# rubengooj/stvo-pl

Hardware: AMD Instinct MI355X
Metric: stereo frames/s (match+optimizePose) (higher is better)
Workload: dtype u8/fp4+f64; 1 GPU; BASELINE configs[2]: KITTI-00-shaped stereo with points + lines (ORB + LBD rows), grid-windowed stereo match (points and lines) + f2f brute-force mutual-NNR match (points and lines) + full GN optimizePose (config_kitti.yaml), device-resident per-frame pipeline; the streams cycle through the 8 sequence ids / 3 KITTI calibrations of configs[4] (sequence s on rank s mod G); streams_per_gpu=3072, parallelism=seq-shard x1

## Files before the change

stvo-pl_amd/csrc/debug_switches.h:

```cpp
#pragma once

#include <climits>

namespace stvo {

constexpr int DBG_UNSET = INT_MIN;

struct DebugSwitches {
    int pose_kernel;
    int pose2p_nw;
    int pose_prof;
    int pose_los;
    int knn_mfma;
    int knn_nseg;
    int seq_inline;
    int line_fused;
    int match_small;
    int match_lazy;
    int grid_tail;
    int grid_fused;
    int grid_fused_cap;
    int lsd_grow;
    int lsd_waves;
    int lsd_xcd_blocks;
    int lsd_feed_ahead;
    int lsd_sep;
    int lsd_multi;
    int lsd_ahead;
    int cells_ahead;
    int lines_ahead;
    int grid_cells;
};

const DebugSwitches& dbg();
void dbg_reparse();

}
```

stvo-pl_amd/csrc/kernels.h:

```cpp
#pragma once

#include <hip/hip_runtime.h>
#include <stdint.h>

#include <cstdlib>
#include <map>
#include <mutex>
#include <utility>

#include "../../include/stvo_hip.h"
#include "debug_switches.h"
#include "point_tail.h"

namespace stvo {

inline bool lds_opt_in(const void* kernel, int bytes) {
    static std::mutex mu;
    static std::map<std::pair<const void*, int>, int> granted;
    int dev = 0;
    if (hipGetDevice(&dev) != hipSuccess) return false;
    std::lock_guard<std::mutex> lk(mu);
    const auto key = std::make_pair(kernel, dev);
    const auto it = granted.find(key);
    if (it != granted.end() && (it->second >= bytes || it->second < 0)) return it->second >= bytes;
// ... 103 lines not shown
    double level_scale;
    const unsigned* wait_flag;
    unsigned wait_value;
    int lazy_eig;
    int lines_on_solver;
    const uint4* fetch_src;
    uint4* fetch_dst;
    unsigned fetch_n16;
    unsigned* fetch_flag;
    unsigned fetch_value;
    unsigned* start_flag;
    unsigned start_value;
};
bool pose_start_flag_ok(const PoseArgs& a);
void launch_stream_gate(hipStream_t s, const unsigned* flag, unsigned value);
constexpr int STVO_POSE_QTAB = 16;
constexpr int PATH_EIG_PENDING = 1 << 30;
bool pose_inline_sync_ok(int B);
void launch_stream_signal(hipStream_t s, unsigned* flag, unsigned value);
int launch_pose(hipStream_t s, const PoseArgs& a);
int launch_pose2p(hipStream_t s, const PoseArgs& a);
bool pose_batch_kernel_selected(const PoseArgs& a);
int pose2p_waves_per_pair(int B);
void pose2p_retain_stream(hipStream_t s);
void pose2p_release_stream(hipStream_t s);

void launch_blur7_u8(hipStream_t s, int B, int cols, int rows, const uint8_t* src, uint8_t* dst, const int* k7);
void launch_resize_linear_u8(hipStream_t s, int B, int scols, int srows, int dcols, int drows, const uint8_t* src, uint8_t* dst, double fx = 0.0,
                             double fy = 0.0);

constexpr int GRID_LW = STVO_GRID_COLS + 16, GRID_LCELLS = STVO_GRID_ROWS * GRID_LW, GRID_LSTART_STRIDE = GRID_LCELLS + 4;
struct PointCells {
    int K, ws;
    const float* kp_l;
    const float* kp_r;
    const int32_t* n_kp_l;
    const int32_t* n_kp_r;
    const double* inv_wh;
    int32_t* pstart;
    uint32_t* plstart;
    int32_t* plperm;
    int32_t* pperm;
    int32_t* pcell;
    int32_t* pxy_l;
    unsigned long long* top2_p;
    int32_t* govf_p;
// ... 60 lines not shown
```

stvo-pl_amd/csrc/pose_block.h:

```cpp
#pragma once
#include <type_traits>

#include "kernels.h"
#include "pose_math.h"

namespace stvo {

namespace {

constexpr int ACT_CONTINUE = 0, ACT_BREAK = 1, ACT_FAIL = 2;

struct PoseSh {
    double DT[16];
    double DT0[16];
    double DT1[16];
    double DTr[16];
    double cov[36];
    double eig[6];
    double H[36];
    double g[6];
    double err, err_prev, err_out, lambda;
    double s_p, s_l;
    unsigned long long xchg[2];
    int action, good, n_inl_p, n_inl_l, n_m_p, n_m_l, evals, itmp;
// ... 195 lines not shown
            const unsigned olo = (unsigned)k_or, ohi = (unsigned)((unsigned long long)k_or >> 32);
            const unsigned a0 = (unsigned)__builtin_amdgcn_update_dpp((int)alo, (int)alo, CTRL, RM, 0xf, false);
            const unsigned a1 = (unsigned)__builtin_amdgcn_update_dpp((int)ahi, (int)ahi, CTRL, RM, 0xf, false);
            const unsigned o0 = (unsigned)__builtin_amdgcn_update_dpp((int)olo, (int)olo, CTRL, RM, 0xf, false);
            const unsigned o1 = (unsigned)__builtin_amdgcn_update_dpp((int)ohi, (int)ohi, CTRL, RM, 0xf, false);
            k_and &= (K)(((unsigned long long)a1 << 32) | a0);
            k_or |= (K)(((unsigned long long)o1 << 32) | o0);
        };
        using std::integral_constant;
        dpp_step(integral_constant<int, 0x111>{}, integral_constant<int, 0xf>{});
        dpp_step(integral_constant<int, 0x112>{}, integral_constant<int, 0xf>{});
        dpp_step(integral_constant<int, 0x114>{}, integral_constant<int, 0xf>{});
        dpp_step(integral_constant<int, 0x118>{}, integral_constant<int, 0xf>{});
        dpp_step(integral_constant<int, 0x142>{}, integral_constant<int, 0xa>{});
        dpp_step(integral_constant<int, 0x143>{}, integral_constant<int, 0xc>{});
        if ((threadIdx.x & 63) == 63) {
            part[0] = (unsigned long long)k_and;
            part[1] = (unsigned long long)k_or;
        }
    }

    template <int NA, int NB, bool W, typename K, int BITS, typename KeyA, typename KeyB>
    static __device__ __forceinline__ void select2(KeyA&& ka, unsigned ma, int ktha, bool acta, KeyB&& kb, unsigned mb, int kthb, bool actb,
                                                   unsigned* S, unsigned long long* xchg, int& rot, K& outa, K& outb, bool sc = false) {
        static_assert(BITS == 32 || BITS == 64, "32- or 64-bit keys");
        const int tid = threadIdx.x, wv = tid >> 6;
        const bool own_b = W ? !sc : sc;
        constexpr bool PFA = BITS == 64 && NA >= 8, PFB = BITS == 64 && NB >= 8;
        K anda = 0, ora = ~(K)0, andb = 0, orb = ~(K)0;
        if (PFA || PFB) {
            unsigned long long* part = reinterpret_cast<unsigned long long*>(S + SEL_PART);
            if (W) {
                if (PFA) sel_and_or<NA, K>(ka, ma, part + 4 * wv);
                if (PFB && !sc) sel_and_or<NB, K>(kb, mb, part + 4 * wv + 2);
            }
            __syncthreads();
            unsigned long long a0 = ~0ull, o0 = 0ull, a1 = ~0ull, o1 = 0ull;
#pragma unroll
            for (int w = 0; w < NWORK; ++w) {
                if (PFA) { a0 &= part[4 * w]; o0 |= part[4 * w + 1]; }
                if (PFB) { a1 &= part[4 * w + 2]; o1 |= part[4 * w + 3]; }
            }
            if (PFA) { anda = (K)a0; ora = (K)o0; }
            if (PFB && !sc) { andb = (K)a1; orb = (K)o1; }
        }
        auto top_bit = [](K differ) -> int {
            return differ == 0 ? -1 : (BITS - 1) - (BITS == 64 ? __clzll((unsigned long long)differ) : __clz((unsigned)differ));
        };
        K pa = anda, pb = andb;
        int kka = ktha, kkb = kthb;
        int hia = acta ? top_bit(anda ^ ora) : -1, hib = actb ? top_bit(andb ^ orb) : -1;
        bool penda = false, pendb = false;
        auto count = [&](auto n_c, auto&& key, unsigned mask, K prefix, int hi, int lo, unsigned* h) {
            constexpr int N = decltype(n_c)::value;
#pragma unroll
            for (int k = 0; k < N; ++k) {
                const K kv = key(k);
                const K diff = kv ^ prefix;
                const bool same = hi + 1 >= BITS ? true : (diff >> (hi + 1 >= BITS ? 0 : hi + 1)) == 0;
// ... 9 lines not shown
            prefix = (prefix & ~((K)127 << lo)) | ((K)bin << lo);
            kk -= below;
            hi = lo - 1;
            if (cnt == 1 && lo > 0) {
                if (own) {
#pragma unroll
                    for (int k = 0; k < N; ++k) {
                        const K kv = key(k);
                        if (((mask >> k) & 1u) && ((kv ^ prefix) >> lo) == 0) *mail = (unsigned long long)kv;
                    }
                }
                pend = true;
                hi = -1;
            }
        };
        using std::integral_constant;
        while (hia >= 0 || hib >= 0) {
            const int loa = hia >= 6 ? hia - 6 : 0, lob = hib >= 6 ? hib - 6 : 0;
            unsigned* const ha = S + rot * SEL_HW;
            unsigned* const hb = S + (3 + rot) * SEL_HW;
            if (W && hia >= 0) count(integral_constant<int, NA>{}, ka, ma, pa, hia, loa, ha);
            if (own_b && hib >= 0) count(integral_constant<int, NB>{}, kb, mb, pb, hib, lob, hb);
            __syncthreads();
            if (W && tid < 2 * SEL_HW) {
                const int rc = rot == 0 ? 2 : rot - 1;
                S[((tid >> 6) * 3 + rc) * SEL_HW + (tid & 63)] = 0u;
            }
            if (hia >= 0) decide(integral_constant<int, NA>{}, W, ka, ma, ha, pa, kka, hia, loa, penda, xchg);
            if (hib >= 0) decide(integral_constant<int, NB>{}, own_b, kb, mb, hb, pb, kkb, hib, lob, pendb, xchg + 1);
            rot = rot == 2 ? 0 : rot + 1;
        }
        __syncthreads();
        if (penda) pa = (K)xchg[0];
        if (pendb) pb = (K)xchg[1];
        if (acta) outa = pa;
        if (actb) outb = pb;
    }

    template <int NA, int NB, bool W>
    static __device__ __forceinline__ void mad_sigma2(const double* va, unsigned ma, int na, const double* vb, unsigned mb, int nb, unsigned* S,
                                                      unsigned long long* xchg, int& rot, double& sa, double& sb, bool sc = false) {
        sa = 0.0;
        sb = 0.0;
        const bool acta = na != 0, actb = nb != 0;
        if (!acta && !actb) return;
        auto image = [](double v) -> unsigned long long {
            const unsigned long long b = (unsigned long long)__double_as_longlong(v);
            return (b >> 63) ? ~b : (b | 0x8000000000000000ull);
        };
        auto value = [](unsigned long long k) -> double {
            return __longlong_as_double((long long)((k >> 63) ? (k & 0x7FFFFFFFFFFFFFFFull) : ~k));
        };
        unsigned long long ra = 0ull, rb = 0ull;
        select2<NA, NB, W, unsigned long long, 64>([&](int k) { return image(va[k]); }, ma, na / 2, acta, [&](int k) { return image(vb[k]); }, mb,
                                                   nb / 2, actb, S, xchg, rot, ra, rb, sc);
        const double meda = value(ra), medb = value(rb);
        unsigned qa = 0u, qb = 0u;
        select2<NA, NB, W, unsigned, 32>([&](int k) { return __float_as_uint(fabsf((float)(va[k] - meda))); }, ma, na / 2, acta,
                                         [&](int k) { return __float_as_uint(fabsf((float)(vb[k] - medb))); }, mb, nb / 2, actb, S, xchg, rot, qa, qb, sc);
        if (acta) sa = 1.4826 * (double)__uint_as_float(qa);
        if (actb) sb = 1.4826 * (double)__uint_as_float(qb);
    }

    template <int N, bool W>
    static __device__ __forceinline__ void sum_at(const double* v, double (*red)[28], int slot0, double* out, bool sc = false) {
        const int lane = threadIdx.x & 63, wv = W ? (int)(threadIdx.x >> 6) : NW;
        if (W || sc) {
#pragma unroll
            for (int k = 0; k < N; ++k) {
                const double s = wave_sum_lane63(v[k]);
                if (lane == 63) red[wv][slot0 + k] = s;
            }
        }
        __syncthreads();
#pragma unroll
        for (int k = 0; k < N; ++k) {
            double s = red[0][slot0 + k];
#pragma unroll
            for (int w = 1; w < NW; ++w) s += red[w][slot0 + k];
            if (sc) s += red[NW][slot0 + k];
            out[k] = s;
        }
    }

    template <int NA, int NB, bool W>
    static __device__ __forceinline__ void outlier_cut(const double* ra, unsigned ma, int na, bool do_a, const double* rb, unsigned mb, int nb,
                                                       bool do_b, double inlier_k, unsigned& inla, unsigned& inlb, unsigned* S,
                                                       unsigned long long* xchg, int& rot, double (*red)[28], int* cnt, bool sc = false) {
        const bool own_b = W ? !sc : sc;
        double sa, sb;
        mad_sigma2<NA, NB, W>(ra, do_a ? ma : 0u, do_a ? na : 0, rb, do_b ? mb : 0u, do_b ? nb : 0, S, xchg, rot, sa, sb, sc);
        double v[6] = {0.0, 0.0, 0.0, 0.0, 0.0, 0.0};
        if (W) {
#pragma unroll
            for (int k = 0; k < NA; ++k)
                if (do_a && ((ma >> k) & 1u)) {
                    if (ra[k] < 2.0 * sa) {
                        v[0] += ra[k];
                        v[1] += 1.0;
                    }
                    v[2] += ra[k];
                }
        }
        if (own_b) {
#pragma unroll
            for (int k = 0; k < NB; ++k)
                if (do_b && ((mb >> k) & 1u)) {
                    if (rb[k] < 2.0 * sb) {
                        v[3] += rb[k];
                        v[4] += 1.0;
                    }
                    v[5] += rb[k];
                }
        }
// ... 176 lines not shown
    for (int i = 0; i < 36; ++i) C[i] = sh->cov[i];
    pm::eig6_ql(C, w);
#pragma unroll
    for (int i = 0; i < 6; ++i) sh->eig[i] = w[i];
    sh->good = pm::is_good_solution(DT, w, err) ? 1 : 0;
}

__device__ __forceinline__ void t0_is_good_fast(PoseSh* sh, const double* DT, double err) {
    if (err < 0.0 || err > 1.0 || !pm::all_finite16(DT)) {
        sh->good = 0;
        return;
    }
    double C[36];
#pragma unroll
    for (int i = 0; i < 36; ++i) C[i] = sh->cov[i];
    if (pm::spd_unit_certificate(C) == 1) {
        sh->good = 1;
        return;
    }
    t0_is_good(sh, DT, err);
}

__device__ __forceinline__ void t0_commit(PoseSh* sh, stvo_pose_result* out, int status, int path, int it0, int it1, bool lazy_eig = false,
                                          double* next_T = nullptr) {
    bool eig_pending = false;
    if (lazy_eig) {
        double C[36];
#pragma unroll
        for (int i = 0; i < 36; ++i) C[i] = sh->cov[i];
        if (sh->err_out < 0.0 || sh->err_out > 1.0 || !pm::all_finite16(sh->DT)) {
            sh->good = 0;
        } else if (pm::spd_unit_certificate(C) == 1) {
            sh->good = 1;
            eig_pending = true;
        } else {
            t0_is_good(sh, sh->DT, sh->err_out);
        }
    } else {
        t0_is_good(sh, sh->DT, sh->err_out);
    }
    double DT[16];
#pragma unroll
    for (int i = 0; i < 16; ++i) {
        DT[i] = sh->DT[i];
        out->T_opt[i] = DT[i];
    }
    out->err_opt = sh->err_out;
    if (sh->good && !pm::is_identity16(DT)) {
        double Ti[16], x[6], T[16];
        pm::inverse_se3(DT, Ti);
        pm::logmap_se3(Ti, x);
        pm::expmap_se3(x, T);
#pragma unroll
        for (int i = 0; i < 16; ++i) out->T[i] = T[i];
        if (next_T) {
            const bool fin = pm::all_finite16(T);
#pragma unroll
            for (int i = 0; i < 16; ++i) next_T[i] = fin ? T[i] : ((i % 5 == 0) ? 1.0 : 0.0);
        }
#pragma unroll
        for (int i = 0; i < 36; ++i) out->cov[i] = sh->cov[i];
#pragma unroll
        for (int i = 0; i < 6; ++i) out->cov_eig[i] = eig_pending ? 0.0 : sh->eig[i];
// ... 132 lines not shown
```

stvo-pl_amd/csrc/pose_kernel2p.hip:

```cpp
#include <cstdlib>

#include <map>
#include <mutex>
#include <utility>
#include <vector>

#include "pose_block.h"

namespace stvo {
namespace {

__device__ __forceinline__ double uni(double v) {
    const long long b = __double_as_longlong(v);
    const int lo = __builtin_amdgcn_readfirstlane((int)(b & 0xFFFFFFFFll)), hi = __builtin_amdgcn_readfirstlane((int)(b >> 32));
    return __longlong_as_double(((long long)hi << 32) | (unsigned long long)(unsigned)lo);
}

struct PointRec2 {
    double X, Y, Z, ox, oy, q;
};

constexpr bool POSE2P_PRIO = true;

template <int NW, bool PROF>
// ... 415 lines not shown
    KArgs* const kargs = (KArgs*)__builtin_amdgcn_kernarg_segment_ptr();
    auto ka = [&]() -> KArgs& {
        KArgs* p = kargs;
        asm volatile("" : "+s"(p));
        return *p;
    };

    constexpr int BLOCK = NW * 64;
    constexpr int PPT = (STVO_POSE_MAX_POINTS + BLOCK - 1) / BLOCK;
    constexpr int LPT = (STVO_POSE_MAX_LINES + BLOCK - 1) / BLOCK;
    constexpr int KL = pose2c_planes<NW>();
    constexpr bool HAS_REG = KL < PPT;
    static_assert(KL <= PPT && PPT <= 16, "4-bit levels of 16 ordinals in one 64-bit word");
    using Ops = BlockOps<NW>;
    extern __shared__ float4 s_ra[];
    double* const s_rb = reinterpret_cast<double*>(s_ra + KL * BLOCK);
    __shared__ __align__(16) int s_hist[2][Ops::HIST_W];
    __shared__ double s_red[NW][28];
    __shared__ int s_ired[NW];
    __shared__ PoseSh s_sh;
    PoseSh* sh = &s_sh;
    const int f = blockIdx.x, tid = threadIdx.x, lane = tid & 63, wv = tid >> 6;
    const bool w0 = wv == 0, t0 = tid == 0;
    long long rprof[3] = {0, 0, 0};
    long long tprof[5] = {0, 0, 0, 0, 0};
    long long wprof[3] = {0, 0, 0}, wave_busy = 0;
    auto tick = [&]() -> long long {
        if constexpr (PROF) return (long long)__builtin_readcyclecounter();
        else return 0ll;
    };
    const long long t_begin = tick();
    if (blockIdx.x == 0 && threadIdx.x == 0 && ka().start_flag)
        __hip_atomic_store(ka().start_flag, ka().start_value, __ATOMIC_RELEASE, __HIP_MEMORY_SCOPE_AGENT);
    stvo_cam cam_f;
    if (ka().cams) {
        cam_f = ka().cams[f];
    } else {
        cam_f.fx = ka().cam.fx; cam_f.fy = ka().cam.fy; cam_f.cx = ka().cam.cx; cam_f.cy = ka().cam.cy; cam_f.b = ka().cam.b;
    }
    const pm::Cam5 cam{cam_f.fx, cam_f.fy, cam_f.cx, cam_f.cy};
    const double cam_b = cam_f.b;
    const double homog_th = ka().prm.homog_th, inv_homog = 1.0 / homog_th;

    unsigned pmatched = 0u, pinl = 0u;
    const int n_prev_p = ka().n_prev_pts != nullptr ? min(ka().n_prev_pts[f], ka().max_pts) : 0;
    const size_t pbase = (size_t)f * ka().max_pts;
    int jj[PPT];
// ... 27 lines not shown
        int initl[LPT];
#pragma unroll
        for (int k = 0; k < LPT; ++k) {
            const int li = li0 + k * BLOCK;
            const int lc = (li < n_prev_l && li < ka().max_lines) ? li : 0;
            jl[k] = (ka().m12l && ka().max_lines > 0) ? ka().m12l[lbase + lc] : lc;
            initl[k] = (ka().init_inl_l && ka().max_lines > 0) ? ka().init_inl_l[lbase + lc] : 1;
        }
#pragma unroll
        for (int k = 0; k < LPT; ++k) {
            const int li = li0 + k * BLOCK;
            if (li < n_prev_l && li < ka().max_lines && jl[k] >= 0) {
                lmatched |= 1u << k;
                if (initl[k] != 0) linl |= 1u << k;
            } else {
                jl[k] = 0;
            }
        }
    }
    const int n_mine = __popc(pmatched);
    unsigned* const sel = reinterpret_cast<unsigned*>(&s_hist[0][0]);
    int sel_rot = 0;
    for (int i = tid; i < 2 * Ops::HIST_W; i += BLOCK) sel[i] = 0u;
    const int n_m_p = Ops::template sum_int<true>(n_mine, s_ired);
    const int n_m_l = Ops::template sum_int<true>(__popc(lmatched), s_ired);

    const unsigned m_o = n_mine >= 32 ? 0xFFFFFFFFu : ((1u << n_mine) - 1u);
    unsigned inl_o = 0u, slow_o = 0u;
    unsigned long long lv = 0ull;
    float4 xa = make_float4(0.f, 0.f, 0.f, 0.f);
    double xb = 1.0;
    {
        int r = 0;
        constexpr int STAGE_CH = PPT;
#pragma unroll
        for (int k0 = 0; k0 < PPT; k0 += STAGE_CH) {
            float4 pv[STAGE_CH], cv[STAGE_CH];
#pragma unroll
            for (int c = 0; c < STAGE_CH; ++c) {
                const int k = k0 + c;
                if (k >= PPT) continue;
                const int ik = tid + k * BLOCK;
                pv[c] = ka().prev_rc[pbase + (size_t)(ik < n_prev_p ? ik : 0)];
                cv[c] = ka().curr_rc[pbase + (size_t)jj[k]];
            }
#pragma unroll
            for (int c = 0; c < STAGE_CH; ++c) {
                const int k = k0 + c;
// ... 35 lines not shown
        const double2 v0 = q[0], v1 = q[BLOCK], v2 = q[2 * BLOCK], v3 = q[3 * BLOCK], v4 = q[4 * BLOCK], v5 = q[5 * BLOCK], v6 = q[6 * BLOCK];
        L.sP[0] = v0.x; L.sP[1] = v0.y; L.sP[2] = v1.x; L.eP[0] = v1.y; L.eP[1] = v2.x; L.eP[2] = v2.y;
        L.le[0] = v3.x; L.le[1] = v3.y; L.le[2] = v4.x; L.spl[0] = v4.y; L.spl[1] = v5.x; L.epl[0] = v5.y; L.epl[1] = v6.x;
        L.sigma2 = v6.y;
        return L;
    };
#pragma unroll
    for (int k = 0; k < LPT; ++k)
        if ((lmatched >> k) & 1u) {
            const size_t i = lbase + (size_t)(li0 + k * BLOCK);
            const size_t j = lbase + (size_t)jl[k];
            const int r = __popc(lmatched & ((1u << k) - 1u));
            double2* q = ar_l + (size_t)(r * 7) * BLOCK + tid;
            q[0] = make_double2(ka().prev_sP[i * 3 + 0], ka().prev_sP[i * 3 + 1]);
            q[BLOCK] = make_double2(ka().prev_sP[i * 3 + 2], ka().prev_eP[i * 3 + 0]);
            q[2 * BLOCK] = make_double2(ka().prev_eP[i * 3 + 1], ka().prev_eP[i * 3 + 2]);
            q[3 * BLOCK] = make_double2(ka().curr_le[j * 3 + 0], ka().curr_le[j * 3 + 1]);
            q[4 * BLOCK] = make_double2(ka().curr_le[j * 3 + 2], ka().prev_spl[i * 2 + 0]);
            q[5 * BLOCK] = make_double2(ka().prev_spl[i * 2 + 1], ka().prev_epl[i * 2 + 0]);
            q[6 * BLOCK] = make_double2(ka().prev_epl[i * 2 + 1], sqrt(ka().prev_s2l[i]));
        }

    {
        const int nip = Ops::template sum_int<true>(__popc(inl_o), s_ired);
        const int nil = Ops::template sum_int<true>(__popc(linl), s_ired);
        if (w0) {
            sh->n_m_p = n_m_p;
            sh->n_m_l = n_m_l;
            sh->n_inl_p = nip;
            sh->n_inl_l = nil;
            sh->good = 1;
            sh->err_out = -1.0;
#pragma unroll
            for (int i = 0; i < 16; ++i) {
                const double v = ka().init_T ? ka().init_T[(size_t)f * 16 + i] : ((i % 5 == 0) ? 1.0 : 0.0);
                sh->DT[i] = v;
                sh->DT0[i] = v;
            }
#pragma unroll
            for (int i = 0; i < 36; ++i) {
                sh->cov[i] = 0.0;
                sh->H[i] = 0.0;
            }
        }
        __syncthreads();
    }
    const long long t_prologue = tick() - t_begin;

    auto rebuild = [&](const float4& av, double bd, double* X, double* Y, double* Z, double* ox, double* oy) {
#pragma clang fp contract(off)
        *X = bd * ((double)av.x - cam_f.cx);
        *Y = bd * ((double)av.y - cam_f.cy);
        *Z = bd * cam_f.fx;
        *ox = (double)av.z;
        *oy = (double)av.w;
    };
    const double* const qtab = ka().q_tab;
    auto q_of = [&](unsigned nib) -> double { return qtab[nib]; };
    auto fetch_slow = [&](int r) -> CompactRec {
        return pose2c_fetch_slow(ka().prev_rc, ka().curr_rc, ka().m12p, pbase, tid, BLOCK, pmatched, r, cam_b, ka().level_scale);
// ... 109 lines not shown
        wave_busy += tw2 - tw0;
        __syncthreads();
        if (w0) {
            if (lane < 28) {
                double sum = s_red[0][lane];
#pragma unroll
                for (int w = 1; w < NW; ++w) sum += s_red[w][lane];
                store_total(sh, lane, sum);
            }
            __builtin_amdgcn_fence(__ATOMIC_RELEASE, "wavefront");
            __builtin_amdgcn_wave_barrier();
            __builtin_amdgcn_fence(__ATOMIC_ACQUIRE, "wavefront");
        }
        wprof[0] += tw1 - tw0;
        wprof[1] += tw2 - tw1;
        wprof[2] += tick() - tw2;
    };

    auto compact_inliers = [&]() {
        unsigned char* const s_lvb = reinterpret_cast<unsigned char*>(&s_hist[0][0]);
        static_assert(sizeof(s_hist) >= (size_t)KL * BLOCK, "the level bytes of a full set of planes fit the histogram scratch");
        const unsigned mov = inl_o & ~slow_o;
        const int c = __popc(mov);
        int incl = c;
#pragma unroll
        for (int off = 1; off < 64; off <<= 1) {
            const int o = __shfl_up(incl, off, 64);
            if (lane >= off) incl += o;
        }
        const int n_slow = Ops::template sum_int<true>(__popc(inl_o & slow_o), s_ired);
        if (lane == 63) s_ired[wv] = incl;
        __syncthreads();
        int base = incl - c, total = 0;
#pragma unroll
        for (int w = 0; w < NW; ++w) {
            const int cw = s_ired[w];
            if (w < wv) base += cw;
            total += cw;
        }
        __syncthreads();
        if (n_slow != 0 || total > KL * BLOCK) return;
        RecRegs<HAS_REG ? KL + 1 : KL> regs;
        auto take = [&](auto rc) {
            constexpr int R = decltype(rc)::value;
            if constexpr (R < KL) {
                regs.template a<R>() = *reinterpret_cast<const f4_native*>(&s_ra[R * BLOCK + tid]);
                regs.template b<R>() = s_rb[R * BLOCK + tid];
            } else {
                regs.template a<R>() = f4_native{xa.x, xa.y, xa.z, xa.w};
                regs.template b<R>() = xb;
            }
        };
        static_for<0, HAS_REG ? KL + 1 : KL>(take);
        __syncthreads();
        {
            int g = base;
            auto put = [&](auto rc) {
                constexpr int R = decltype(rc)::value;
                if ((mov >> R) & 1u) {
                    *reinterpret_cast<f4_native*>(&s_ra[g]) = regs.template a<R>();
                    s_rb[g] = regs.template b<R>();
                    s_lvb[g] = (unsigned char)((lv >> (4 * R)) & 15u);
                    ++g;
                }
            };
            static_for<0, HAS_REG ? KL + 1 : KL>(put);
        }
        __syncthreads();
        const int n_hold = tid < total ? (total - tid + BLOCK - 1) / BLOCK : 0;
        unsigned long long lvn = 0ull;
#pragma unroll
        for (int r = 0; r < KL; ++r)
            if (r < n_hold) lvn |= (unsigned long long)s_lvb[r * BLOCK + tid] << (4 * r);
        lv = lvn;
        inl_w = n_hold > 0 ? ((1u << n_hold) - 1u) : 0u;
        dealt = true;
        const int first = wv * 64;
        n_trip = first < total ? (total - first + BLOCK - 1) / BLOCK : 0;
        __syncthreads();
        for (int i = tid; i < 2 * Ops::HIST_W; i += BLOCK) sel[i] = 0u;
        __syncthreads();
    };

    auto remove_outliers = [&]() {
        double DT[12];
        pose_sgpr(sh->DT1, DT);
        const bool do_p = ka().prm.has_points != 0, do_l = ka().prm.has_lines != 0;
        const long long tr0 = tick();
        double resp[PPT], resl[LPT];
        residuals(DT, do_p ? m_o : 0u, true, resp);
#pragma unroll
        for (int k = 0; k < LPT; ++k) {
            resl[k] = 0.0;
            if (do_l && ((lmatched >> k) & 1u)) {
                const pm::LineRec L = load_line(k);
                resl[k] = pm::line_residual(DT, cam, L) * L.sigma2;
            }
        }
        const long long tr1 = tick();
        int cnt[2];
        Ops::template outlier_cut<PPT, LPT, true>(resp, m_o, sh->n_m_p, do_p, resl, lmatched, sh->n_m_l, do_l, ka().prm.inlier_k, inl_o, linl, sel,
                                                  sh->xchg, sel_rot, s_red, cnt);
        if (w0) {
            if (do_p) sh->n_inl_p = cnt[0];
            if (do_l) sh->n_inl_l = cnt[1];
        }
        __syncthreads();
        const long long tr2 = tick();
        compact_inliers();
        rprof[0] += tr1 - tr0;
        rprof[1] += tr2 - tr1;
        rprof[2] += tick() - tr2;
    };

    auto params = [&]() -> const stvo_opt_params __attribute__((address_space(4)))& { return ka().prm; };
    const PoseFlow fl = optimize_pose_flow<POSE2P_PRIO>(sh, params, w0, evaluate, remove_outliers, tick, tprof, &s_red[0][0]);

    {
        const long long tq3 = tick();
        if (t0) t0_commit(sh, ka().results + f, fl.status, fl.path, fl.it0, fl.it1, false, ka().next_T ? ka().next_T + (size_t)f * 16 : nullptr);
        tprof[2] += tick() - tq3;
    }
    if (PROF && t0) {
        tprof[4] = tick() - t_begin;
#pragma unroll
        for (int i = 0; i < 5; ++i) ka().prof_out[(size_t)f * 16 + i] = tprof[i];
#pragma unroll
        for (int i = 0; i < 3; ++i) ka().prof_out[(size_t)f * 16 + 5 + i] = wprof[i];
        ka().prof_out[(size_t)f * 16 + 14] = t_prologue;
#pragma unroll
        for (int i = 0; i < 3; ++i) ka().prof_out[(size_t)f * 16 + 10 + i] = rprof[i];
    }
    if (PROF && lane == 0 && (wv < 6 || wv == NW - 1)) ka().prof_out[(size_t)f * 16 + 8 + (wv < 6 ? wv : 7)] = wave_busy;

    if (ka().inl_p_out) {
        const size_t base = (size_t)f * ka().max_pts;
#pragma unroll
        for (int k = 0; k < PPT; ++k) {
            const int i = tid + k * BLOCK;
            const int r = __popc(pmatched & ((1u << k) - 1u));
            if (i < ka().max_pts) ka().inl_p_out[base + i] = ((pmatched >> k) & 1u) ? (int)((inl_o >> r) & 1u) : -1;
        }
    }
    if (ka().inl_l_out && ka().max_lines > 0) {
#pragma unroll
        for (int k = 0; k < LPT; ++k) {
            const int li = li0 + k * BLOCK;
            if (li < ka().max_lines) ka().inl_l_out[(size_t)f * ka().max_lines + li] = ((lmatched >> k) & 1u) ? (int)((linl >> k) & 1u) : -1;
        }
    }
}

struct ArenaBuf {
    double2* dev = nullptr;
    size_t bytes = 0;
    int users = 0;
    std::vector<void*> retired;
};

std::mutex g_arena_mu;
std::map<std::pair<int, hipStream_t>, ArenaBuf> g_arenas;

double2* arena_ptr(hipStream_t s, size_t bytes) {
    int dev = 0;
    if (hipGetDevice(&dev) != hipSuccess) return nullptr;
    std::lock_guard<std::mutex> lk(g_arena_mu);
    ArenaBuf& b = g_arenas[std::make_pair(dev, s)];
    if (b.bytes < bytes || !b.dev) {
        if (b.dev) b.retired.push_back(b.dev);
        b.dev = nullptr;
        b.bytes = 0;
        if (hipMalloc((void**)&b.dev, bytes > 256 ? bytes : 256) != hipSuccess) return nullptr;
        b.bytes = bytes;
// ... 49 lines not shown
    int dev = 0;
    if (hipGetDevice(&dev) != hipSuccess) return;
    std::lock_guard<std::mutex> lk(g_arena_mu);
    ++g_arenas[std::make_pair(dev, s)].users;
}

void pose2p_release_stream(hipStream_t s) {
    int dev = 0;
    if (hipGetDevice(&dev) != hipSuccess) return;
    std::lock_guard<std::mutex> lk(g_arena_mu);
    const auto it = g_arenas.find(std::make_pair(dev, s));
    if (it == g_arenas.end()) return;
    if (--it->second.users > 0) return;
    if (it->second.dev) (void)hipFree(it->second.dev);
    for (void* p : it->second.retired) (void)hipFree(p);
    g_arenas.erase(it);
}

int pose2p_waves_per_pair(int B) {
    const int nw = dbg().pose2p_nw != DBG_UNSET && dbg().pose2p_nw > 0 ? dbg().pose2p_nw : (B > 2 * device_cu_count() ? 2 : 4);
    return nw >= 4 ? 4 : 2;
}

int launch_pose2p(hipStream_t s, const PoseArgs& a) {
    if (a.B <= 0) return STVO_OK;
    if (a.eval_only) return STVO_ERR_INVALID_ARG;
    if (a.max_pts > STVO_POSE_MAX_POINTS || a.max_lines > STVO_POSE_MAX_LINES) return STVO_ERR_CAPACITY;
    if (a.prev_rc && (!a.curr_rc || !a.q_tab)) return STVO_ERR_INVALID_ARG;
    const int nw = pose2p_waves_per_pair(a.B);
    if (a.prev_rc) return nw == 4 ? launch_pose2c_variant<4>(s, a, 2) : launch_pose2c_variant<2>(s, a, 4);
    return nw == 4 ? launch_pose2p_variant<4>(s, a, 2) : launch_pose2p_variant<2>(s, a, 4);
}

}
```

stvo-pl_amd/csrc/seq_pipeline.hip:

```cpp
#include <algorithm>
#include <atomic>
#include <chrono>
#include <cstdio>
#include <cstdlib>
#include <vector>

#include "ctx_internal.h"
#include "point_cells.h"
#include "pose_math.h"
#include "step_plan.h"

#pragma clang fp contract(off)

namespace stvo {
namespace {

constexpr int LENT = STVO_GRID_COLS + STVO_GRID_ROWS + 4;

struct SeqDev {
    int B, K, M;
    const stvo_cam* cams;
    const double* inv_wh;
    stvo_match_params mp;
    const float* kp_l;
// ... 1187 lines not shown
    std::memset(&a, 0, sizeof(a));
    a.B = B; a.max_pts = s->K; a.max_lines = s->M;
    a.n_prev_pts = s->op.has_points ? ps.n : nullptr;
    a.prev_rc = ps.rc; a.curr_rc = cs.rc; a.q_tab = s->d_qtab; a.level_scale = s->mp.orb_scale_factor; a.m12p = s->m12p;
    a.n_prev_lines = s->op.has_lines ? ps.nl : nullptr;
    a.prev_sP = ps.sP; a.prev_eP = ps.eP; a.prev_spl = ps.spl; a.prev_epl = ps.epl; a.prev_s2l = ps.s2lm;
    a.curr_le = cs.le; a.m12l = m12l_use;
    a.cams = s->d_cams; a.prm = s->op;
    a.init_T = s->d_motion_T; a.next_T = s->d_motion_T;
    a.results = s->zero_copy ? reinterpret_cast<stvo_pose_result*>(s->out_host) : s->results;
    a.inl_p_out = s->inlp; a.inl_l_out = s->inll;
    if (p.inl_zero_copy) {
        a.inl_p_out = reinterpret_cast<int32_t*>(s->fetch_host + s->m12_span);
        a.inl_l_out = reinterpret_cast<int32_t*>(s->fetch_host + s->m12_span + (reinterpret_cast<const char*>(s->inll) - reinterpret_cast<const char*>(s->inlp)));
    }
    if (stvo::dbg().pose_prof != stvo::DBG_UNSET) {
        if (!s->d_prof) HIP_TRY(ctx, hipMalloc((void**)&s->d_prof, (size_t)B * 16 * sizeof(long long)));
        a.prof_out = s->d_prof;
    }
    if (p.join_signal) {
        a.wait_flag = s->d_join_flag;
        a.wait_value = s->join_epoch;
    }
    a.lazy_eig = p.lazy_eig ? 1 : 0;
    if (p.fetch_by_pose) {
        a.fetch_src = reinterpret_cast<const uint4*>(s->m12s_p);
        a.fetch_dst = reinterpret_cast<uint4*>(s->fetch_host);
        a.fetch_n16 = (unsigned)(s->m12_span / 16);
        a.fetch_flag = reinterpret_cast<unsigned*>(s->fetch_host + s->m12_span + s->inl_span);
        a.fetch_value = pub.fetch_value = ++s->fetch_epoch;
    }
    if (p.pose_flagged) {
        a.start_flag = s->d_pose_flag;
        a.start_value = pub.pose_flag_value = ++s->pose_epoch;
    }
    mark(8, st);
    TRY(stvo::launch_pose(st, a));
    mark(9, st);
    if (ctl)
        stvo::launch_stream_ctl_post(st, B, ctl, a.results, s->d_motion_T, s->fetch ? a.inl_p_out : nullptr, s->K, s->fetch ? a.inl_l_out : nullptr, s->M);
    if (p.inl_copy) stvo::launch_copy16(st, s->inlp, s->fetch_host + s->m12_span, s->inl_span);
    return STVO_OK;
}

int seq_enqueue_step(stvo_seq* s, int slot, const StepFlags& fl, stvo::StepPlan& plan, StepPub& pub) {
    stvo_ctx* ctx = s->ctx;
    hipEvent_t* tev = nullptr;
    if (s->timing) {
        while (s->tev.size() < s->tev_used + 2 * STVO_SEQ_NSTAGE) {
            hipEvent_t e;
            if (hipEventCreate(&e) != hipSuccess) break;
            s->tev.push_back(e);
        }
        if (s->tev.size() >= s->tev_used + 2 * STVO_SEQ_NSTAGE) {
            tev = s->tev.data() + s->tev_used;
            s->tev_used += 2 * STVO_SEQ_NSTAGE;
        }
    }
    pub = StepPub{};
    stvo_seq::Set& cs = s->set[s->cur];
    stvo::SeqDev d = s->d;
// ... 201 lines not shown
int stvo_seq_restart_fast_dev(stvo_seq* s, int32_t* th_dev, int th0) {
    if (!s || !th_dev || th0 < 1 || th0 > 254) return STVO_ERR_INVALID_ARG;
    if (!s->ctl_staged) return STVO_OK;
    stvo_ctx* ctx = s->ctx;
    HIP_TRY(ctx, hipSetDevice(ctx->device));
    stvo::launch_fast_restart(ctx->stream, s->B, s->d_ctl[s->ctl_next], th_dev, th0);
    return check_launch(ctx);
}

int stvo_seq_read(stvo_seq* s, stvo_pose_result* results, int32_t* counts) {
    if (!s) return STVO_ERR_INVALID_ARG;
    stvo_ctx* ctx = s->ctx;
    HIP_TRY(ctx, hipSetDevice(ctx->device));
    const int B = s->B;
    hipStream_t st = ctx->stream;
    const stvo_seq::Set& ls = s->set[s->prev_set()];
    if (s->d_prof && s->frame_idx > 1) {
        HIP_TRY(ctx, hipStreamSynchronize(st));
        std::vector<long long> h((size_t)B * 16);
        HIP_TRY(ctx, hipMemcpy(h.data(), s->d_prof, h.size() * sizeof(long long), hipMemcpyDeviceToHost));
        double m[16] = {0, 0, 0, 0, 0, 0, 0, 0, 0, 0, 0, 0, 0, 0, 0, 0};
        for (int f = 0; f < B; ++f)
            for (int i = 0; i < 16; ++i) m[i] += (double)h[(size_t)f * 16 + i] / B;
        std::fprintf(stderr, "[pose prof] mean ticks/pair: evaluate %.0f  iter-algebra %.0f  cov+isgood+commit %.0f  remove_outliers %.0f  total %.0f | "
                             "eval-compute %.0f  fold %.0f  barrier+sum %.0f | prologue %.0f | wave busy %.0f %.0f | removeOutliers: residuals %.0f  statistics %.0f  re-deal %.0f\n",
                     m[0], m[1], m[2], m[3], m[4], m[5], m[6], m[7], m[14], m[8], m[9], m[10], m[11], m[12]);
    }
    const bool track = s->frame_idx > 1;
    char* OH = s->out_host;
    const size_t res_bytes = (size_t)B * sizeof(stvo_pose_result);
    if (!s->zero_copy) {
        if (track) HIP_TRY(ctx, hipMemcpyAsync(OH, s->results, res_bytes, hipMemcpyDeviceToHost, st));
        HIP_TRY(ctx, hipMemcpyAsync(OH + res_bytes, ls.n, (size_t)B * 4, hipMemcpyDeviceToHost, st));
        HIP_TRY(ctx, hipMemcpyAsync(OH + res_bytes + (size_t)B * 4, ls.nl, (size_t)B * 4, hipMemcpyDeviceToHost, st));
    }
    HIP_TRY(ctx, hipStreamSynchronize(st));
    s->uploads_done = s->uploads;
    s->st_dirty = false;
    const stvo_pose_result* hr = reinterpret_cast<const stvo_pose_result*>(OH);
    const int32_t* hn = reinterpret_cast<const int32_t*>(OH + res_bytes);
    for (int b = 0; b < B; ++b) {
        if (results) {
            if (track) {
                results[b] = hr[b];
                if (results[b].path & stvo::PATH_EIG_PENDING) {
                    pm::eig6_ql(results[b].cov, results[b].cov_eig);
                    results[b].path &= ~stvo::PATH_EIG_PENDING;
                }
            }
// ... 249 lines not shown
```

stvo-pl_amd/csrc/step_plan.h:

```cpp
#pragma once

#include <algorithm>
#include <cstddef>
#include <cstdint>

#include "../../include/stvo_hip.h"
#include "debug_switches.h"

namespace stvo {

constexpr int LSF_MAX_LINES = 512, LSF_BYTES_PER_LINE = 32 + 16 + 16 + 4 + 2 * STVO_GRID_ROWS + 2 + 2 + 1;

inline DebugSwitches switches_unset() {
    static_assert(sizeof(DebugSwitches) % sizeof(int) == 0, "DebugSwitches holds ints only");
    DebugSwitches d;
    int* v = reinterpret_cast<int*>(&d);
    for (size_t k = 0; k < sizeof(d) / sizeof(int); ++k) v[k] = DBG_UNSET;
    return d;
}

struct StepFacts {
    int B = 0, K = 0, M = 0, cus = 0;
    bool has_points = false, has_lines = false, best_lr_matches = false;
    bool lines_now = false, lines_prev = false, track = false;
// ... 33 lines not shown
};

struct StepPlan {
    bool light = false;
    bool par = false;
    bool mid_fork = false;
    bool fork_at_start = false;
    bool line_forked = false;
    bool zero_nl = false;
    bool point_stage = false, line_stage = false;
    bool clear_nl = false;
    bool lean_cells = false, has_tail = false, fused_cells = false, cells_ahead = false, lines_ahead = false, gate = false;
    int Mk = 0;
    size_t line_lds = 0;
    bool line_fused = false;
    MatchPlan match_points, match_lines;
    bool track = false;
    bool match_lines_run = false, clear_m12l = false;
    bool use_alt_m12l = false;
    bool inline_sync = false, fetch_by_pose = false, inl_zero_copy = false, lazy_eig = false, pose_flagged = false;
    bool join_signal = false;
    bool fetch_copy = false;
    bool inl_copy = false;
    int32_t schedule[8] = {0, 0, 0, 0, 0, 0, 0, 0};
};

template <class LdsFits>
inline StepPlan plan_step(const StepFacts& f, const StepHistory& h, LdsFits&& lds_fits) {
    StepPlan p;
    const int B = f.B;
    const long long last = f.frame_idx - 1;
    const bool tev = f.timing != 0 && f.timing_events;
    p.light = tev && f.timing == 2;
    const bool alt_ok = f.has_alt_m12l && !f.fetch;
    p.use_alt_m12l = alt_ok && (f.frame_idx & 1);
    p.par = f.lines_now && f.has_points;
    p.mid_fork = p.par && B >= 64;
    const bool fork_free = p.par && f.raw_split && !f.st_dirty && !f.has_control;
    p.fork_at_start = p.par && !p.mid_fork && !fork_free;
    p.line_forked = p.par && (p.mid_fork || !fork_free);
    p.zero_nl = !f.lines_now && f.has_points;
    p.point_stage = f.has_points;
    p.line_stage = f.lines_now;
    p.clear_nl = !f.lines_now && !p.zero_nl;
    p.track = f.track;

// ... 25 lines not shown
        auto route = [&](bool small_ok, bool timed, int small_cap) {
            MatchPlan m;
            if (small_ok && small_sets && !timed) {
                m.route = MatchRoute::SMALL;
                m.small_cap = small_cap;
            } else if (f.best_lr_matches && B <= 4 && !timed && !elz) {
                m.route = MatchRoute::BOTH_DIRS;
                m.nseg_cap = 4;
            } else {
                m.route = f.best_lr_matches ? MatchRoute::LAZY : MatchRoute::ONE_WAY;
            }
            return m;
        };
        p.match_points = route(f.match_small_ok_K, tev, 0);
        p.match_lines = route(f.match_small_ok_M, false, lines_cap);
        p.match_lines_run = f.lines_prev && f.lines_now;
        p.clear_m12l = f.lines_prev && !f.lines_now;
        p.inline_sync = f.pose_inline_sync_ok && f.sw.seq_inline != 0 && !tev && (!f.fetch || (B == 1 && f.zero_copy));
        p.join_signal = p.par && p.inline_sync;
        p.fetch_by_pose = f.fetch && p.inline_sync;
        p.inl_zero_copy = f.fetch && f.zero_copy;
        p.inl_copy = f.fetch && !p.inl_zero_copy;
        p.lazy_eig = p.inline_sync && f.zero_copy && f.sw.pose_kernel != 4;
        p.pose_flagged = f.has_alt_m12l && f.pose_start_flag_ok;
        p.schedule[STVO_SCHED_POSE_KERNEL] = f.pose_batch_kernel_selected ? STVO_SCHED_POSE_BATCH : STVO_SCHED_POSE_LATENCY;
        p.schedule[STVO_SCHED_POSE_WAVES] = f.pose_batch_kernel_selected ? f.pose2p_waves_per_pair : 0;
    }
    p.fetch_copy = f.fetch && !p.fetch_by_pose;
    p.schedule[STVO_SCHED_FUSED_CELLS] = p.fused_cells;
    p.schedule[STVO_SCHED_CELLS_AHEAD] = p.cells_ahead;
    p.schedule[STVO_SCHED_LINES_AHEAD] = p.lines_ahead;
    p.schedule[STVO_SCHED_GATE] = p.gate;
    p.schedule[STVO_SCHED_MID_FORK] = p.mid_fork;
    p.schedule[STVO_SCHED_LINE_FUSED] = p.line_fused;
    return p;
}

inline void commit(StepHistory& h, const StepPlan& p, long long frame_idx) {
    if (p.mid_fork) h.fork_rec_frame = frame_idx;
    if (p.pose_flagged) h.pose_flag_frame = frame_idx;
    if (p.line_forked) h.sl_forked_frame = frame_idx;
}

}
```

stvo-pl_amd/csrc/stvo_capi.hip:

```cpp
#include <hip/hip_runtime.h>

#include <cstdio>
#include <cstdlib>
#include <cstring>
#include <new>
#include <vector>

#include "ctx_internal.h"

namespace stvo {
namespace {

int env_int(const char* name) {
    const char* e = std::getenv(name);
    return (e && *e) ? std::atoi(e) : DBG_UNSET;
}
DebugSwitches parse_switches() {
    DebugSwitches d;
    d.pose_kernel = env_int("STVO_POSE_KERNEL");
    d.pose2p_nw = env_int("STVO_POSE2P_NW");
    d.pose_prof = env_int("STVO_POSE_PROF");
    d.pose_los = env_int("STVO_POSE_LOS");
    d.knn_mfma = env_int("STVO_KNN_MFMA");
    d.knn_nseg = env_int("STVO_KNN_NSEG");
    d.seq_inline = env_int("STVO_SEQ_INLINE");
    d.cells_ahead = env_int("STVO_CELLS_AHEAD");
    d.line_fused = env_int("STVO_LINE_FUSED");
    d.match_small = env_int("STVO_MATCH_SMALL");
    d.match_lazy = env_int("STVO_MATCH_LAZY");
    d.grid_tail = env_int("STVO_GRID_TAIL");
    d.grid_fused = env_int("STVO_GRID_FUSED");
    d.grid_fused_cap = env_int("STVO_GRID_FUSED_CAP");
    d.grid_cells = env_int("STVO_GRID_CELLS");
    d.lines_ahead = env_int("STVO_LINES_AHEAD");
    d.lsd_grow = env_int("STVO_LSD_GROW");
    d.lsd_waves = env_int("STVO_LSD_WAVES");
    d.lsd_xcd_blocks = env_int("STVO_LSD_XCD_BLOCKS");
    d.lsd_feed_ahead = env_int("STVO_LSD_FEED_AHEAD");
    d.lsd_sep = env_int("STVO_LSD_SEP");
    d.lsd_ahead = env_int("STVO_LSD_AHEAD");
    d.lsd_multi = env_int("STVO_LSD_MULTI");
    return d;
}
DebugSwitches& switches() {
    static DebugSwitches d = parse_switches();
    return d;
}

}

const DebugSwitches& dbg() { return switches(); }
void dbg_reparse() { switches() = parse_switches(); }

}

extern "C" {

// ... 544 lines not shown
```

Measured before the change: 1.386 million frame-pairs/s.

## Offload pose covariance eigen-decomposition to a separate kernel and merge block reductions

```diff
diff --git a/stvo-pl_amd/csrc/debug_switches.h b/stvo-pl_amd/csrc/debug_switches.h
--- a/stvo-pl_amd/csrc/debug_switches.h
+++ b/stvo-pl_amd/csrc/debug_switches.h
@@ -29,6 +29,7 @@
     int lsd_ahead;
     int cells_ahead;
     int lines_ahead;
+    int pose_eig;
     int grid_cells;
 };
 
diff --git a/stvo-pl_amd/csrc/kernels.h b/stvo-pl_amd/csrc/kernels.h
--- a/stvo-pl_amd/csrc/kernels.h
+++ b/stvo-pl_amd/csrc/kernels.h
@@ -149,6 +149,7 @@
 int launch_pose2p(hipStream_t s, const PoseArgs& a);
 bool pose_batch_kernel_selected(const PoseArgs& a);
 int pose2p_waves_per_pair(int B);
+void launch_pose_eig(hipStream_t s, stvo_pose_result* results, int B);
 void pose2p_retain_stream(hipStream_t s);
 void pose2p_release_stream(hipStream_t s);
 
diff --git a/stvo-pl_amd/csrc/pose_block.h b/stvo-pl_amd/csrc/pose_block.h
--- a/stvo-pl_amd/csrc/pose_block.h
+++ b/stvo-pl_amd/csrc/pose_block.h
@@ -241,8 +241,11 @@
 
     template <int NA, int NB, bool W, typename K, int BITS, typename KeyA, typename KeyB>
     static __device__ __forceinline__ void select2(KeyA&& ka, unsigned ma, int ktha, bool acta, KeyB&& kb, unsigned mb, int kthb, bool actb,
-                                                   unsigned* S, unsigned long long* xchg, int& rot, K& outa, K& outb, bool sc = false) {
+                                                   unsigned* S, unsigned long long* xchg, int& rot, K& outa, K& outb, bool sc = false,
+                                                   int* stat = nullptr) {
         static_assert(BITS == 32 || BITS == 64, "32- or 64-bit keys");
+        int* const st = stat ? stat + (BITS == 64 ? 0 : 4) : nullptr;
+        if (st) ++st[0];
         const int tid = threadIdx.x, wv = tid >> 6;
         const bool own_b = W ? !sc : sc;
         constexpr bool PFA = BITS == 64 && NA >= 8, PFB = BITS == 64 && NB >= 8;
@@ -254,6 +257,7 @@
                 if (PFB && !sc) sel_and_or<NB, K>(kb, mb, part + 4 * wv + 2);
             }
             __syncthreads();
+            if (st) ++st[3];
             unsigned long long a0 = ~0ull, o0 = 0ull, a1 = ~0ull, o1 = 0ull;
 #pragma unroll
             for (int w = 0; w < NWORK; ++w) {
@@ -309,6 +313,11 @@
             if (W && hia >= 0) count(integral_constant<int, NA>{}, ka, ma, pa, hia, loa, ha);
             if (own_b && hib >= 0) count(integral_constant<int, NB>{}, kb, mb, pb, hib, lob, hb);
             __syncthreads();
+            if (st) {
+                st[1] += hia >= 0;
+                st[2] += hib >= 0;
+                ++st[3];
+            }
             if (W && tid < 2 * SEL_HW) {
                 const int rc = rot == 0 ? 2 : rot - 1;
                 S[((tid >> 6) * 3 + rc) * SEL_HW + (tid & 63)] = 0u;
@@ -318,6 +327,7 @@
             rot = rot == 2 ? 0 : rot + 1;
         }
         __syncthreads();
+        if (st) ++st[3];
         if (penda) pa = (K)xchg[0];
         if (pendb) pb = (K)xchg[1];
         if (acta) outa = pa;
@@ -326,7 +336,8 @@
 
     template <int NA, int NB, bool W>
     static __device__ __forceinline__ void mad_sigma2(const double* va, unsigned ma, int na, const double* vb, unsigned mb, int nb, unsigned* S,
-                                                      unsigned long long* xchg, int& rot, double& sa, double& sb, bool sc = false) {
+                                                      unsigned long long* xchg, int& rot, double& sa, double& sb, bool sc = false,
+                                                      int* stat = nullptr) {
         sa = 0.0;
         sb = 0.0;
         const bool acta = na != 0, actb = nb != 0;
@@ -340,11 +351,11 @@
         };
         unsigned long long ra = 0ull, rb = 0ull;
         select2<NA, NB, W, unsigned long long, 64>([&](int k) { return image(va[k]); }, ma, na / 2, acta, [&](int k) { return image(vb[k]); }, mb,
-                                                   nb / 2, actb, S, xchg, rot, ra, rb, sc);
+                                                   nb / 2, actb, S, xchg, rot, ra, rb, sc, stat);
         const double meda = value(ra), medb = value(rb);
         unsigned qa = 0u, qb = 0u;
         select2<NA, NB, W, unsigned, 32>([&](int k) { return __float_as_uint(fabsf((float)(va[k] - meda))); }, ma, na / 2, acta,
-                                         [&](int k) { return __float_as_uint(fabsf((float)(vb[k] - medb))); }, mb, nb / 2, actb, S, xchg, rot, qa, qb, sc);
+                                         [&](int k) { return __float_as_uint(fabsf((float)(vb[k] - medb))); }, mb, nb / 2, actb, S, xchg, rot, qa, qb, sc, stat);
         if (acta) sa = 1.4826 * (double)__uint_as_float(qa);
         if (actb) sb = 1.4826 * (double)__uint_as_float(qb);
     }
@@ -373,10 +384,11 @@
     template <int NA, int NB, bool W>
     static __device__ __forceinline__ void outlier_cut(const double* ra, unsigned ma, int na, bool do_a, const double* rb, unsigned mb, int nb,
                                                        bool do_b, double inlier_k, unsigned& inla, unsigned& inlb, unsigned* S,
-                                                       unsigned long long* xchg, int& rot, double (*red)[28], int* cnt, bool sc = false) {
+                                                       unsigned long long* xchg, int& rot, double (*red)[28], int* cnt, bool sc = false,
+                                                       int* stat = nullptr) {
         const bool own_b = W ? !sc : sc;
         double sa, sb;
-        mad_sigma2<NA, NB, W>(ra, do_a ? ma : 0u, do_a ? na : 0, rb, do_b ? mb : 0u, do_b ? nb : 0, S, xchg, rot, sa, sb, sc);
+        mad_sigma2<NA, NB, W>(ra, do_a ? ma : 0u, do_a ? na : 0, rb, do_b ? mb : 0u, do_b ? nb : 0, S, xchg, rot, sa, sb, sc, stat);
         double v[6] = {0.0, 0.0, 0.0, 0.0, 0.0, 0.0};
         if (W) {
 #pragma unroll
@@ -599,8 +611,9 @@
 }
 
 __device__ __forceinline__ void t0_commit(PoseSh* sh, stvo_pose_result* out, int status, int path, int it0, int it1, bool lazy_eig = false,
-                                          double* next_T = nullptr) {
+                                          double* next_T = nullptr, long long* eig_ticks = nullptr) {
     bool eig_pending = false;
+    const long long te0 = eig_ticks ? (long long)__builtin_readcyclecounter() : 0ll;
     if (lazy_eig) {
         double C[36];
 #pragma unroll
@@ -616,6 +629,7 @@
     } else {
         t0_is_good(sh, sh->DT, sh->err_out);
     }
+    if (eig_ticks) *eig_ticks = (long long)__builtin_readcyclecounter() - te0;
     double DT[16];
 #pragma unroll
     for (int i = 0; i < 16; ++i) {
diff --git a/stvo-pl_amd/csrc/pose_kernel2p.hip b/stvo-pl_amd/csrc/pose_kernel2p.hip
--- a/stvo-pl_amd/csrc/pose_kernel2p.hip
+++ b/stvo-pl_amd/csrc/pose_kernel2p.hip
@@ -461,7 +461,12 @@
     PoseSh* sh = &s_sh;
     const int f = blockIdx.x, tid = threadIdx.x, lane = tid & 63, wv = tid >> 6;
     const bool w0 = wv == 0, t0 = tid == 0;
-    long long rprof[3] = {0, 0, 0};
+    long long rprof[3] = {0, 0, 0}, eig_ticks = 0;
+    int sstat_cut[8] = {0, 0, 0, 0, 0, 0, 0, 0};
+    auto sel_stat = [&]() -> int* {
+        if constexpr (PROF) return sstat_cut;
+        else return nullptr;
+    };
     long long tprof[5] = {0, 0, 0, 0, 0};
     long long wprof[3] = {0, 0, 0}, wave_busy = 0;
     auto tick = [&]() -> long long {
@@ -535,8 +540,13 @@
     unsigned* const sel = reinterpret_cast<unsigned*>(&s_hist[0][0]);
     int sel_rot = 0;
     for (int i = tid; i < 2 * Ops::HIST_W; i += BLOCK) sel[i] = 0u;
-    const int n_m_p = Ops::template sum_int<true>(n_mine, s_ired);
-    const int n_m_l = Ops::template sum_int<true>(__popc(lmatched), s_ired);
+    int n_tot[4];
+    {
+        const int n_own[4] = {n_mine, (int)__popc(lmatched), (int)__popc(pinl), (int)__popc(linl)};
+        Ops::template sum_int4<true>(n_own, s_red, n_tot);
+    }
+    double t_init = (lane % 5 == 0) ? 1.0 : 0.0;
+    if (w0 && lane < 16 && ka().init_T) t_init = ka().init_T[(size_t)f * 16 + lane];
 
     const unsigned m_o = n_mine >= 32 ? 0xFFFFFFFFu : ((1u << n_mine) - 1u);
     unsigned inl_o = 0u, slow_o = 0u;
@@ -618,20 +628,16 @@
         }
 
     {
-        const int nip = Ops::template sum_int<true>(__popc(inl_o), s_ired);
-        const int nil = Ops::template sum_int<true>(__popc(linl), s_ired);
         if (w0) {
-            sh->n_m_p = n_m_p;
-            sh->n_m_l = n_m_l;
-            sh->n_inl_p = nip;
-            sh->n_inl_l = nil;
+            sh->n_m_p = n_tot[0];
+            sh->n_m_l = n_tot[1];
+            sh->n_inl_p = n_tot[2];
+            sh->n_inl_l = n_tot[3];
             sh->good = 1;
             sh->err_out = -1.0;
-#pragma unroll
-            for (int i = 0; i < 16; ++i) {
-                const double v = ka().init_T ? ka().init_T[(size_t)f * 16 + i] : ((i % 5 == 0) ? 1.0 : 0.0);
-                sh->DT[i] = v;
-                sh->DT0[i] = v;
+            if (lane < 16) {
+                sh->DT[lane] = t_init;
+                sh->DT0[lane] = t_init;
             }
 #pragma unroll
             for (int i = 0; i < 36; ++i) {
@@ -787,23 +793,22 @@
         static_assert(sizeof(s_hist) >= (size_t)KL * BLOCK, "the level bytes of a full set of planes fit the histogram scratch");
         const unsigned mov = inl_o & ~slow_o;
         const int c = __popc(mov);
-        int incl = c;
+        int incl = c | (__popc(inl_o & slow_o) << 16);
 #pragma unroll
         for (int off = 1; off < 64; off <<= 1) {
             const int o = __shfl_up(incl, off, 64);
             if (lane >= off) incl += o;
         }
-        const int n_slow = Ops::template sum_int<true>(__popc(inl_o & slow_o), s_ired);
         if (lane == 63) s_ired[wv] = incl;
         __syncthreads();
-        int base = incl - c, total = 0;
+        int base = (incl & 0xFFFF) - c, total = 0, n_slow = 0;
 #pragma unroll
         for (int w = 0; w < NW; ++w) {
             const int cw = s_ired[w];
-            if (w < wv) base += cw;
-            total += cw;
-        }
-        __syncthreads();
+            if (w < wv) base += cw & 0xFFFF;
+            total += cw & 0xFFFF;
+            n_slow += cw >> 16;
+        }
         if (n_slow != 0 || total > KL * BLOCK) return;
         RecRegs<HAS_REG ? KL + 1 : KL> regs;
         auto take = [&](auto rc) {
@@ -844,7 +849,6 @@
         n_trip = first < total ? (total - first + BLOCK - 1) / BLOCK : 0;
         __syncthreads();
         for (int i = tid; i < 2 * Ops::HIST_W; i += BLOCK) sel[i] = 0u;
-        __syncthreads();
     };
 
     auto remove_outliers = [&]() {
@@ -865,12 +869,11 @@
         const long long tr1 = tick();
         int cnt[2];
         Ops::template outlier_cut<PPT, LPT, true>(resp, m_o, sh->n_m_p, do_p, resl, lmatched, sh->n_m_l, do_l, ka().prm.inlier_k, inl_o, linl, sel,
-                                                  sh->xchg, sel_rot, s_red, cnt);
+                                                  sh->xchg, sel_rot, s_red, cnt, false, sel_stat());
         if (w0) {
             if (do_p) sh->n_inl_p = cnt[0];
             if (do_l) sh->n_inl_l = cnt[1];
         }
-        __syncthreads();
         const long long tr2 = tick();
         compact_inliers();
         rprof[0] += tr1 - tr0;
@@ -883,7 +886,8 @@
 
     {
         const long long tq3 = tick();
-        if (t0) t0_commit(sh, ka().results + f, fl.status, fl.path, fl.it0, fl.it1, false, ka().next_T ? ka().next_T + (size_t)f * 16 : nullptr);
+        if (t0) t0_commit(sh, ka().results + f, fl.status, fl.path, fl.it0, fl.it1, ka().lazy_eig != 0, ka().next_T ? ka().next_T + (size_t)f * 16 : nullptr,
+                          PROF ? &eig_ticks : nullptr);
         tprof[2] += tick() - tq3;
     }
     if (PROF && t0) {
@@ -892,9 +896,12 @@
         for (int i = 0; i < 5; ++i) ka().prof_out[(size_t)f * 16 + i] = tprof[i];
 #pragma unroll
         for (int i = 0; i < 3; ++i) ka().prof_out[(size_t)f * 16 + 5 + i] = wprof[i];
-        ka().prof_out[(size_t)f * 16 + 14] = t_prologue;
+        ka().prof_out[(size_t)f * 16 + 14] = t_prologue | (eig_ticks << 32);
 #pragma unroll
         for (int i = 0; i < 3; ++i) ka().prof_out[(size_t)f * 16 + 10 + i] = rprof[i];
+        auto pack4 = [](const int* v) -> long long { return (long long)v[0] | ((long long)v[1] << 16) | ((long long)v[2] << 32) | ((long long)v[3] << 48); };
+        ka().prof_out[(size_t)f * 16 + 13] = pack4(sstat_cut);
+        ka().prof_out[(size_t)f * 16 + 15] = pack4(sstat_cut + 4);
     }
     if (PROF && lane == 0 && (wv < 6 || wv == NW - 1)) ka().prof_out[(size_t)f * 16 + 8 + (wv < 6 ? wv : 7)] = wave_busy;
 
@@ -914,6 +921,22 @@
             if (li < ka().max_lines) ka().inl_l_out[(size_t)f * ka().max_lines + li] = ((lmatched >> k) & 1u) ? (int)((linl >> k) & 1u) : -1;
         }
     }
+}
+
+constexpr int POSE_EIG_WAVES = 4;
+__global__ __launch_bounds__(POSE_EIG_WAVES * 64) void pose_eig_kernel(stvo_pose_result* results, int B) {
+    const int b = blockIdx.x * POSE_EIG_WAVES + (int)(threadIdx.x >> 6);
+    if (b >= B || (threadIdx.x & 63) != 0) return;
+    stvo_pose_result* r = results + b;
+    const int path = r->path;
+    if (!(path & PATH_EIG_PENDING)) return;
+    double C[36], w[6];
+#pragma unroll
+    for (int i = 0; i < 36; ++i) C[i] = r->cov[i];
+    pm::eig6_ql(C, w);
+#pragma unroll
+    for (int i = 0; i < 6; ++i) r->cov_eig[i] = w[i];
+    r->path = path & ~PATH_EIG_PENDING;
 }
 
 struct ArenaBuf {
@@ -1009,6 +1032,11 @@
     return nw >= 4 ? 4 : 2;
 }
 
+void launch_pose_eig(hipStream_t s, stvo_pose_result* results, int B) {
+    if (B <= 0) return;
+    hipLaunchKernelGGL(pose_eig_kernel, dim3((B + POSE_EIG_WAVES - 1) / POSE_EIG_WAVES), dim3(POSE_EIG_WAVES * 64), 0, s, results, B);
+}
+
 int launch_pose2p(hipStream_t s, const PoseArgs& a) {
     if (a.B <= 0) return STVO_OK;
     if (a.eval_only) return STVO_ERR_INVALID_ARG;
diff --git a/stvo-pl_amd/csrc/seq_pipeline.hip b/stvo-pl_amd/csrc/seq_pipeline.hip
--- a/stvo-pl_amd/csrc/seq_pipeline.hip
+++ b/stvo-pl_amd/csrc/seq_pipeline.hip
@@ -1233,7 +1233,7 @@
         a.wait_flag = s->d_join_flag;
         a.wait_value = s->join_epoch;
     }
-    a.lazy_eig = p.lazy_eig ? 1 : 0;
+    a.lazy_eig = (p.lazy_eig || p.eig_kernel) ? 1 : 0;
     if (p.fetch_by_pose) {
         a.fetch_src = reinterpret_cast<const uint4*>(s->m12s_p);
         a.fetch_dst = reinterpret_cast<uint4*>(s->fetch_host);
@@ -1248,6 +1248,7 @@
     mark(8, st);
     TRY(stvo::launch_pose(st, a));
     mark(9, st);
+    if (p.eig_kernel) stvo::launch_pose_eig(st, a.results, B);
     if (ctl)
         stvo::launch_stream_ctl_post(st, B, ctl, a.results, s->d_motion_T, s->fetch ? a.inl_p_out : nullptr, s->K, s->fetch ? a.inl_l_out : nullptr, s->M);
     if (p.inl_copy) stvo::launch_copy16(st, s->inlp, s->fetch_host + s->m12_span, s->inl_span);
@@ -1495,9 +1496,22 @@
         double m[16] = {0, 0, 0, 0, 0, 0, 0, 0, 0, 0, 0, 0, 0, 0, 0, 0};
         for (int f = 0; f < B; ++f)
             for (int i = 0; i < 16; ++i) m[i] += (double)h[(size_t)f * 16 + i] / B;
+        double pro = 0.0, eig = 0.0, sel[8] = {0, 0, 0, 0, 0, 0, 0, 0};
+        for (int f = 0; f < B; ++f) {
+            const unsigned long long w14 = (unsigned long long)h[(size_t)f * 16 + 14];
+            pro += (double)(w14 & 0xFFFFFFFFull) / B;
+            eig += (double)(w14 >> 32) / B;
+            for (int i = 0; i < 8; ++i)
+                sel[i] += (double)(((unsigned long long)h[(size_t)f * 16 + (i < 4 ? 13 : 15)] >> (16 * (i & 3))) & 0xFFFFull) / B;
+        }
+        m[14] = pro;
         std::fprintf(stderr, "[pose prof] mean ticks/pair: evaluate %.0f  iter-algebra %.0f  cov+isgood+commit %.0f  remove_outliers %.0f  total %.0f | "
                              "eval-compute %.0f  fold %.0f  barrier+sum %.0f | prologue %.0f | wave busy %.0f %.0f | removeOutliers: residuals %.0f  statistics %.0f  re-deal %.0f\n",
                      m[0], m[1], m[2], m[3], m[4], m[5], m[6], m[7], m[14], m[8], m[9], m[10], m[11], m[12]);
+        if (s->last_schedule[STVO_SCHED_POSE_KERNEL] == STVO_SCHED_POSE_BATCH)
+            std::fprintf(stderr, "[pose prof] of the commit: eig6_ql %.0f | selections of removeOutliers, mean per pair: 64-bit keys: calls %.2f  rounds "
+                                 "key-points %.2f  key-lines %.2f  barriers %.2f | 32-bit keys: calls %.2f  rounds key-points %.2f  key-lines %.2f  "
+                                 "barriers %.2f\n", eig, sel[0], sel[1], sel[2], sel[3], sel[4], sel[5], sel[6], sel[7]);
     }
     const bool track = s->frame_idx > 1;
     char* OH = s->out_host;
diff --git a/stvo-pl_amd/csrc/step_plan.h b/stvo-pl_amd/csrc/step_plan.h
--- a/stvo-pl_amd/csrc/step_plan.h
+++ b/stvo-pl_amd/csrc/step_plan.h
@@ -79,6 +79,7 @@
     bool join_signal = false;
     bool fetch_copy = false;
     bool inl_copy = false;
+    bool eig_kernel = false;
     int32_t schedule[8] = {0, 0, 0, 0, 0, 0, 0, 0};
 };
 
@@ -150,6 +151,8 @@
         p.inl_zero_copy = f.fetch && f.zero_copy;
         p.inl_copy = f.fetch && !p.inl_zero_copy;
         p.lazy_eig = p.inline_sync && f.zero_copy && f.sw.pose_kernel != 4;
+        const bool eig_safe = f.pose_batch_kernel_selected && !f.fetch && f.timing == 0;
+        p.eig_kernel = eig_safe && f.sw.pose_eig != 0 && (f.sw.pose_eig == 1 || B > 8 * f.cus);
         p.pose_flagged = f.has_alt_m12l && f.pose_start_flag_ok;
         p.schedule[STVO_SCHED_POSE_KERNEL] = f.pose_batch_kernel_selected ? STVO_SCHED_POSE_BATCH : STVO_SCHED_POSE_LATENCY;
         p.schedule[STVO_SCHED_POSE_WAVES] = f.pose_batch_kernel_selected ? f.pose2p_waves_per_pair : 0;
diff --git a/stvo-pl_amd/csrc/stvo_capi.hip b/stvo-pl_amd/csrc/stvo_capi.hip
--- a/stvo-pl_amd/csrc/stvo_capi.hip
+++ b/stvo-pl_amd/csrc/stvo_capi.hip
@@ -33,6 +33,7 @@
     d.grid_fused_cap = env_int("STVO_GRID_FUSED_CAP");
     d.grid_cells = env_int("STVO_GRID_CELLS");
     d.lines_ahead = env_int("STVO_LINES_AHEAD");
+    d.pose_eig = env_int("STVO_POSE_EIG");
     d.lsd_grow = env_int("STVO_LSD_GROW");
     d.lsd_waves = env_int("STVO_LSD_WAVES");
     d.lsd_xcd_blocks = env_int("STVO_LSD_XCD_BLOCKS");
```

Result: faster. 1.405 million frame-pairs/s (median of 6 runs) (+1.3%).
